# caoql98/LKGD

Hardware: AMD Instinct MI355X
Metric: denoised frames/sec (14f x 576x1024, 25-step Euler) (higher is better)
Workload: dtype f16; 1 GPU; SVD 14 frames x 576x1024, 25 Euler steps, CFG 1.0->3.0, single clip, vanilla pipeline_stable_video_diffusion_trans loop (configs[1]); unet=random-init SVD shapes (320,640,1280,1280), heads (5,10,20,20), 1.52 B params, parallelism=single GPU

## Files before the change

### include/lkgd_hip.h

```cpp
#ifndef LKGD_HIP_H
#define LKGD_HIP_H

#include <stddef.h>
#include <stdint.h>

#ifdef __cplusplus
extern "C" {
#endif

typedef void* lkgd_stream_t;

enum {
  LKGD_OK = 0,
  LKGD_E_NULL = -1,
  LKGD_E_SHAPE = -2,
  LKGD_E_ALIGN = -3,
  LKGD_E_MODE = -4,
  LKGD_E_LAUNCH = -5
};

enum { LKGD_A_PLAIN = 0, LKGD_A_CONV3X3 = 1, LKGD_A_TCONV3 = 2, LKGD_A_CONV3X3_C8 = 3, LKGD_A_CCONV3 = 4 };

typedef struct lkgd_gemm_desc {
  const void* a0;
// ... 64 lines not shown
                   float eps, const void* rowbias, int32_t ldrb, int32_t rb_d1, int32_t rb_m1, int32_t rb_d2,
                   int32_t rb_md, void* out, int32_t ldo, lkgd_stream_t stream);

int lkgd_tattn_block_c320(const void* x, int32_t ldx, const void* wstream, const float* bo, const void* rowbias, int32_t ldrb,
                          int32_t rb_d1, int32_t rb_m1, int32_t rb_d2, int32_t rb_md, int32_t rb_c0, void* out, int32_t ldo,
                          int32_t B, int32_t F, int32_t HW, float eps, lkgd_stream_t stream);

int lkgd_ln_qkv_c320(const void* x, int32_t ldx, int64_t T, const void* wstream, float eps, void* out, int32_t ldo,
                     lkgd_stream_t stream);
int lkgd_ln_qkv_c640(const void* x, int32_t ldx, int64_t T, const void* wstream, float eps, void* out, int32_t ldo,
                     lkgd_stream_t stream);

int lkgd_ff_fused_c320(const void* x, int32_t ldx, int64_t T, const void* rowbias, int32_t ldrb, int32_t rb_d1, int32_t rb_md,
                       const void* wstream, const float* b2, float eps, float s_acc, const void* res2, int32_t ldr2, float r2,
                       void* out, int32_t ldo, lkgd_stream_t stream);

int lkgd_attn_spatial(const void* q, int32_t ldq, const void* k, int32_t ldk, const void* v, int32_t ldv,
                      void* out, int32_t ldo, int32_t nbatch, int32_t S, int32_t heads, const int32_t* kv_batch_map,
                      float scale, lkgd_stream_t stream);
int lkgd_attn_spatial_qk(const void* q, int32_t ldq, const void* k, int32_t ldk, const void* v, int32_t ldv, void* out,
                         int32_t ldo, int32_t nbatch, int32_t Sq, int32_t S, int32_t heads, const int32_t* kv_batch_map,
                         float scale, lkgd_stream_t stream);

int lkgd_attn_temporal(const void* q, int32_t ldq, const void* k, int32_t ldk, const void* v, int32_t ldv,
                       void* out, int32_t ldo, int32_t B, int32_t Fq, int32_t Fk, int32_t S, int32_t heads,
                       const int32_t* kv_b_map, float scale, lkgd_stream_t stream);

int lkgd_tattn_front(const void* x, int32_t ldx, const void* wpack, const float* bqkv, void* out, int32_t ldo, int32_t B,
                     int32_t F, int32_t HW, int32_t heads, float eps, float scale, lkgd_stream_t stream);

int lkgd_prepare_unet_input(const void* latents, int32_t latents_is_f32, const void* image_latents, int32_t B,
                            int32_t F, int32_t H, int32_t W, int32_t cfg, float sigma, void* tokens_out,
                            lkgd_stream_t stream);
int lkgd_cfg_euler_step(const void* noise_tokens, void* latents, int32_t latents_is_f32, const float* guidance,
                        int32_t B, int32_t F, int32_t H, int32_t W, int32_t cfg, float sigma, float sigma_next,
                        int32_t prediction_type , lkgd_stream_t stream);
int lkgd_cfg_fusion_euler_step(const void* noise_tokens, void* latents, int32_t latents_is_f32, const float* guidance,
                               const float* weight, int32_t B, int32_t F, int32_t H, int32_t W, int32_t cfg, float sigma,
                               float sigma_next, int32_t prediction_type , lkgd_stream_t stream);
int lkgd_shard_rows(const void* src, void* dst, int32_t fl, int32_t HW, int32_t C, int32_t k, const int32_t* px, int32_t pack,
                    lkgd_stream_t stream);
int lkgd_tokens_to_nchw(const void* tokens, int32_t ld, int64_t N, int32_t C, int32_t HW, void* out,
                        lkgd_stream_t stream);
int lkgd_nchw_to_tokens(const void* nchw, int64_t N, int32_t C, int32_t HW, void* tokens, int32_t ld,
                        lkgd_stream_t stream);

// ... 65 lines not shown
```

### lkgd_amd/csrc/attn_spatial.hip

```cpp
#include "common.h"

#define KVBLK 64
#ifndef ATT_KVB16
#define ATT_KVB16 128
#endif
#ifndef ATT_NST
#define ATT_NST 2
#endif
#define ATT_THR 5.0f

__device__ __forceinline__ int k_lds_off(int row, int c) { return row * 128 + ((c ^ ((row >> 1) & 7)) << 4); }
__device__ __forceinline__ int v_lds_off(int row, int c) { return row * 128 + ((c ^ (((row >> 1) & 1) << 2)) << 4); }

template <int NW, int KVB>
__global__ __launch_bounds__(NW * 64, NW == 16 ? 1 : 2) void attn_spatial_kernel(const half_t* __restrict__ q, int ldq,
                                                              const half_t* __restrict__ k, int ldk,
                                                              const half_t* __restrict__ v, int ldv,
                                                              half_t* __restrict__ out, int ldo, int Sq, int S, int heads,
                                                              const int* __restrict__ kvmap, float scale_log2e,
                                                              int nqb, int nwg) {
  extern __shared__ __attribute__((aligned(16))) char smem[];
  const int t = threadIdx.x, lane = t & 63, w = t >> 6;
  const int h = lane >> 5, l31 = lane & 31;
  constexpr int STAGE = 2 * KVB * 128;
// ... 244 lines not shown
template <int NW, int KVB>
static int attn_launch(const void* q, int32_t ldq, const void* k, int32_t ldk, const void* v, int32_t ldv, void* out,
                       int32_t ldo, int32_t nbatch, int32_t Sq, int32_t S, int32_t heads, const int32_t* kv_batch_map, float scale,
                       hipStream_t stream) {
  constexpr int LDS = ATT_NST * 2 * KVB * 128;
  LKGD_DEVICE_ONCE_BEGIN
    if (!lkgd_dynamic_lds(LDS, attn_spatial_kernel<NW, KVB>)) return LKGD_E_LAUNCH;
  LKGD_DEVICE_ONCE_END
  const int QBLK = NW * 32;
  const int nqb = (Sq + QBLK - 1) / QBLK;
  const long long nwg = (long long)nqb * nbatch * heads;
  if (nwg > 0x7fffffffLL) return LKGD_E_SHAPE;
  hipLaunchKernelGGL((attn_spatial_kernel<NW, KVB>), dim3((unsigned)nwg), dim3(NW * 64), LDS, stream, (const half_t*)q, ldq,
                     (const half_t*)k, ldk, (const half_t*)v, ldv, (half_t*)out, ldo, Sq, S, heads, kv_batch_map,
                     scale * 1.4426950408889634f, nqb, (int)nwg);
  return hipGetLastError() == hipSuccess ? LKGD_OK : LKGD_E_LAUNCH;
}

extern "C" int lkgd_attn_spatial_qk(const void* q, int32_t ldq, const void* k, int32_t ldk, const void* v, int32_t ldv,
                                    void* out, int32_t ldo, int32_t nbatch, int32_t Sq, int32_t S, int32_t heads,
                                    const int32_t* kv_batch_map, float scale, lkgd_stream_t stream) {
  if (!q || !k || !v || !out) return LKGD_E_NULL;
  if (nbatch <= 0 || S <= 0 || Sq <= 0 || heads <= 0) return LKGD_E_SHAPE;
  if (ldq % 8 || ldk % 8 || ldv % 8 || ldo % 4) return LKGD_E_ALIGN;
  if (ldq < heads * 64 || ldk < heads * 64 || ldv < heads * 64 || ldo < heads * 64) return LKGD_E_SHAPE;
  if (!aligned16(q) || !aligned16(k) || !aligned16(v) || ((uintptr_t)out & 7)) return LKGD_E_ALIGN;
  if (attn_pipe_mode != 1 && S >= 128 && !attn_nw_override && !attn_kvb_override &&
      (attn_pipe_mode == 2 || (S >= 4096 && Sq >= 4096)))
    return lkgd_attn_pipe_launch(q, ldq, k, ldk, v, ldv, out, ldo, nbatch, Sq, S, heads, kv_batch_map, scale,
                                 (hipStream_t)stream);
  const int nw = attn_nw_override ? attn_nw_override : (Sq >= 8192 ? 16 : Sq >= 2304 ? 8 : 4);
  const int kvb = attn_kvb_override ? attn_kvb_override : (nw == 16 ? ATT_KVB16 : 64);
  hipStream_t st = (hipStream_t)stream;
#define ATT_ARGS q, ldq, k, ldk, v, ldv, out, ldo, nbatch, Sq, S, heads, kv_batch_map, scale, st
  if (nw == 16) return kvb == 128 ? attn_launch<16, 128>(ATT_ARGS) : attn_launch<16, 64>(ATT_ARGS);
  if (nw == 8) return kvb == 128 ? attn_launch<8, 128>(ATT_ARGS) : attn_launch<8, 64>(ATT_ARGS);
  return attn_launch<4, 64>(ATT_ARGS);
#undef ATT_ARGS
}

extern "C" int lkgd_attn_spatial(const void* q, int32_t ldq, const void* k, int32_t ldk, const void* v, int32_t ldv,
                                 void* out, int32_t ldo, int32_t nbatch, int32_t S, int32_t heads,
                                 const int32_t* kv_batch_map, float scale, lkgd_stream_t stream) {
  return lkgd_attn_spatial_qk(q, ldq, k, ldk, v, ldv, out, ldo, nbatch, S, S, heads, kv_batch_map, scale, stream);
}
```

### lkgd_amd/csrc/attn_spatial_pipe.hip

```cpp
#include "asm_host.h"
#include "attn_spatial_pipe.inc"
#include "attn_spatial_pipe_masked.inc"

#define AP_NW 8
#define AP_STAGE 32768
#define AP_LDS (3 * AP_STAGE)

template <int BASE>
__device__ __forceinline__ void ap_load_q(const half_t* qp, float scale_log2e) {
  for_n<4>([&](auto ks_) {
    constexpr int ks = decltype(ks_)::value;
    const half8_t raw = *(const half8_t*)(qp + ks * 16);
    half8_t sc;
#pragma unroll
    for (int e = 0; e < 8; ++e) sc[e] = (half_t)((float)raw[e] * scale_log2e);
    typedef unsigned uint4_t __attribute__((ext_vector_type(4)));
    const uint4_t u = __builtin_bit_cast(uint4_t, sc);
    agpr_write<BASE + 4 * ks + 0>(u[0]);
    agpr_write<BASE + 4 * ks + 1>(u[1]);
    agpr_write<BASE + 4 * ks + 2>(u[2]);
    agpr_write<BASE + 4 * ks + 3>(u[3]);
  });
}

template <int OBASE>
__device__ __forceinline__ void ap_store_tile(half_t* op, float inv, bool valid) {
  for_n<2>([&](auto df_) {
    constexpr int df = decltype(df_)::value;
    for_n<4>([&](auto g_) {
      constexpr int g = decltype(g_)::value;
      half4_t o;
      o[0] = (half_t)(agpr_readf<OBASE + 16 * df + 4 * g + 0>() * inv);
      o[1] = (half_t)(agpr_readf<OBASE + 16 * df + 4 * g + 1>() * inv);
      o[2] = (half_t)(agpr_readf<OBASE + 16 * df + 4 * g + 2>() * inv);
      o[3] = (half_t)(agpr_readf<OBASE + 16 * df + 4 * g + 3>() * inv);
      if (valid) *(half4_t*)(op + 32 * df + 8 * g) = o;
    });
  });
}

template <bool MASKED>
__global__ __launch_bounds__(AP_NW * 64, 1) __attribute__((amdgpu_num_vgpr(ATTN_PIPE_VEND))) void attn_pipe_kernel(
    const half_t* __restrict__ q, int ldq, const half_t* __restrict__ k, int ldk, const half_t* __restrict__ v, int ldv,
    half_t* __restrict__ out, int ldo, int Sq, int S, int heads, const int* __restrict__ kvmap, float scale_log2e, int nqb,
    int nwg) {
  extern __shared__ __attribute__((aligned(16))) char smem[];
  const int t = threadIdx.x, lane = t & 63;
  const int w = __builtin_amdgcn_readfirstlane(t >> 6);
  const int h = lane >> 5, l31 = lane & 31;

  int bid = blockIdx.x;
  {
    int xcd = bid & 7, slot = bid >> 3;
    int qq = nwg >> 3, r = nwg & 7;
    bid = (xcd < r ? xcd * (qq + 1) : r * (qq + 1) + (xcd - r) * qq) + slot;
  }
  const int bh = bid / nqb, qb = bid - bh * nqb;
  const int n = bh / heads, head = bh - n * heads;
  const int kvn = kvmap ? kvmap[n] : n;

  const half_t* kbase = k + (long long)kvn * S * ldk + head * 64;
  const half_t* vbase = v + (long long)kvn * S * ldv + head * 64;
  const int srow0 = w * 8 + (lane >> 3), sc = lane & 7;
  const int kc0 = (sc ^ ((srow0 >> 1) & 7)) * 8;
  const int vc0 = (sc ^ (((srow0 >> 1) & 1) << 2)) * 8;
  const unsigned vok = (unsigned)(srow0 * ldk + kc0) * 2u, vov = (unsigned)(srow0 * ldv + vc0) * 2u;
#pragma unroll
  for (int p = 0; p < 2; ++p) {
    char* dst = smem + (p * 64 + w * 8) * 128;
    glds16((const char*)kbase + (size_t)(p * 64) * ldk * 2 + vok, dst);
    glds16((const char*)vbase + (size_t)(p * 64) * ldv * 2 + vov, dst + 16384);
  }

  const int qrowA = qb * (AP_NW * 64) + w * 64 + l31, qrowB = qrowA + 32;
  {
    const int ra = qrowA < Sq ? qrowA : Sq - 1, rb = qrowB < Sq ? qrowB : Sq - 1;
    ap_load_q<ATTN_PIPE_QF_A>(q + ((long long)n * Sq + ra) * ldq + head * 64 + h * 8, scale_log2e);
    ap_load_q<ATTN_PIPE_QF_B>(q + ((long long)n * Sq + rb) * ldq + head * 64 + h * 8, scale_log2e);
  }

  const unsigned lds0 = (unsigned)(uintptr_t)(__attribute__((address_space(3))) char*)smem;
  unsigned ka0, ka1, ka2, ka3, va0, va1;
  {
    const int sw = (l31 >> 1) & 7;
    ka0 = lds0 + l31 * 128 + (((0 + h) ^ sw) << 4);
    ka1 = lds0 + l31 * 128 + (((2 + h) ^ sw) << 4);
    ka2 = lds0 + l31 * 128 + (((4 + h) ^ sw) << 4);
    ka3 = lds0 + l31 * 128 + (((6 + h) ^ sw) << 4);
    const int i16 = lane & 15, dgrp = (lane >> 4) & 1;
    const int tr_row = 4 * h + (i16 >> 2), tr_c = dgrp * 2 + ((i16 & 3) >> 1), tr_sub = (i16 & 1) * 8;
    const int vsw = ((tr_row >> 1) & 1) << 2;
    va0 = lds0 + tr_row * 128 + (((0 + tr_c) ^ vsw) << 4) + tr_sub;
    va1 = lds0 + tr_row * 128 + (((4 + tr_c) ^ vsw) << 4) + tr_sub;
  }
  const unsigned xora = (unsigned)((lane ^ 32) * 4);
  const unsigned hmask = h == 0 ? 0xffffu : 0u;

  const int nstages = MASKED ? (S + 127) / 128 : S / 128;
  const int dup = nstages * 128 - S;
  const int row1 = (MASKED && nstages == 2) ? S - 128 : 128;
  const unsigned long long kp = (unsigned long long)(uintptr_t)kbase + (unsigned long long)row1 * ldk * 2;
  const unsigned long long vp = (unsigned long long)(uintptr_t)vbase + (unsigned long long)row1 * ldv * 2;
  const auto [klo, khi] = sgpr_ptr(kp);
  const auto [vlo, vhi] = sgpr_ptr(vp);
  const unsigned dst1 = __builtin_amdgcn_readfirstlane(lds0 + AP_STAGE + w * 1024);
  const unsigned ldsend = __builtin_amdgcn_readfirstlane(lds0 + 3 * AP_STAGE);
  const unsigned nst = __builtin_amdgcn_readfirstlane((unsigned)nstages);
  const unsigned kp1 = __builtin_amdgcn_readfirstlane((unsigned)(64 * ldk * 2)), vp1 = __builtin_amdgcn_readfirstlane((unsigned)(64 * ldv * 2));
  const unsigned kstr = __builtin_amdgcn_readfirstlane((unsigned)(128 * ldk * 2)), vstr = __builtin_amdgcn_readfirstlane((unsigned)(128 * ldv * 2));

  float la, lb;
  if constexpr (MASKED) {
    const unsigned vm = (unsigned)l31, hm32 = h == 0 ? 0xffffffffu : 0u;
    const unsigned dupk = __builtin_amdgcn_readfirstlane((unsigned)dup);
    const unsigned klast = __builtin_amdgcn_readfirstlane((unsigned)((128 - dup) * ldk * 2));
    const unsigned vlast = __builtin_amdgcn_readfirstlane((unsigned)((128 - dup) * ldv * 2));
    asm volatile(ATTN_PIPEM_ASM
                 : [la] "=&v"(la), [lb] "=&v"(lb), [ka0] "+v"(ka0), [ka1] "+v"(ka1), [ka2] "+v"(ka2), [ka3] "+v"(ka3),
                   [va0] "+v"(va0), [va1] "+v"(va1)
                 : [vok] "v"(vok), [vov] "v"(vov), [xora] "v"(xora), [hmask] "v"(hmask), [vm] "v"(vm), [hm32] "v"(hm32), [klo] "s"(klo), [khi] "s"(khi), [vlo] "s"(vlo), [vhi] "s"(vhi),
                   [dst1] "s"(dst1), [nst] "s"(nst), [kp1] "s"(kp1), [vp1] "s"(vp1), [kstr] "s"(kstr), [vstr] "s"(vstr),
                   [ldsend] "s"(ldsend), [dup] "s"(dupk), [klast] "s"(klast), [vlast] "s"(vlast)
                 : ATTN_PIPEM_CLOBBERS);
  } else {
    asm volatile(ATTN_PIPE_ASM
                 : [la] "=&v"(la), [lb] "=&v"(lb), [ka0] "+v"(ka0), [ka1] "+v"(ka1), [ka2] "+v"(ka2), [ka3] "+v"(ka3),
                   [va0] "+v"(va0), [va1] "+v"(va1)
                 : [vok] "v"(vok), [vov] "v"(vov), [xora] "v"(xora), [hmask] "v"(hmask), [klo] "s"(klo), [khi] "s"(khi),
                   [vlo] "s"(vlo), [vhi] "s"(vhi), [dst1] "s"(dst1), [nst] "s"(nst), [kp1] "s"(kp1), [vp1] "s"(vp1),
                   [kstr] "s"(kstr), [vstr] "s"(vstr), [ldsend] "s"(ldsend)
                 : ATTN_PIPE_CLOBBERS);
  }

  int lane2;
  asm volatile("v_mbcnt_lo_u32_b32 %0, -1, 0\n\tv_mbcnt_hi_u32_b32 %0, -1, %0" : "=v"(lane2));
  const int h2 = lane2 >> 5, l2 = lane2 & 31;
  const float la_t = la + __shfl_xor(la, 32, 64), lb_t = lb + __shfl_xor(lb, 32, 64);
  const int qa = qb * (AP_NW * 64) + w * 64 + l2, qbb = qa + 32;
  const int ra2 = qa < Sq ? qa : Sq - 1, rb2 = qbb < Sq ? qbb : Sq - 1;
  ap_store_tile<ATTN_PIPE_O_A>(out + ((long long)n * Sq + ra2) * ldo + head * 64 + 4 * h2, 1.0f / la_t, qa < Sq);
  ap_store_tile<ATTN_PIPE_O_B>(out + ((long long)n * Sq + rb2) * ldo + head * 64 + 4 * h2, 1.0f / lb_t, qbb < Sq);
}

int lkgd_attn_pipe_launch(const void* q, int32_t ldq, const void* k, int32_t ldk, const void* v, int32_t ldv, void* out,
                          int32_t ldo, int32_t nbatch, int32_t Sq, int32_t S, int32_t heads, const int32_t* kv_batch_map,
                          float scale, hipStream_t stream) {
  if (S < 128) return LKGD_E_SHAPE;
  const bool masked = S % 128 != 0;
  if ((long long)64 * ldk * 2 > 0x7fffffffLL || (long long)64 * ldv * 2 > 0x7fffffffLL) return LKGD_E_SHAPE;
  LKGD_DEVICE_ONCE_BEGIN
    if (!lkgd_dynamic_lds(AP_LDS, attn_pipe_kernel<false>, attn_pipe_kernel<true>)) return LKGD_E_LAUNCH;
  LKGD_DEVICE_ONCE_END
  const int QBLK = AP_NW * 64;
  const int nqb = (Sq + QBLK - 1) / QBLK;
  const long long nwg = (long long)nqb * nbatch * heads;
  if (nwg > 0x7fffffffLL) return LKGD_E_SHAPE;
  if (masked)
    hipLaunchKernelGGL(attn_pipe_kernel<true>, dim3((unsigned)nwg), dim3(AP_NW * 64), AP_LDS, stream, (const half_t*)q, ldq,
                       (const half_t*)k, ldk, (const half_t*)v, ldv, (half_t*)out, ldo, Sq, S, heads, kv_batch_map,
                       scale * 1.4426950408889634f, nqb, (int)nwg);
  else
    hipLaunchKernelGGL(attn_pipe_kernel<false>, dim3((unsigned)nwg), dim3(AP_NW * 64), AP_LDS, stream, (const half_t*)q, ldq,
                       (const half_t*)k, ldk, (const half_t*)v, ldv, (half_t*)out, ldo, Sq, S, heads, kv_batch_map,
                       scale * 1.4426950408889634f, nqb, (int)nwg);
  return hipGetLastError() == hipSuccess ? LKGD_OK : LKGD_E_LAUNCH;
}
```

### lkgd_amd/csrc/qkv_fused.hip

```cpp
#include "asm_host.h"
#include "qkv_fused_loop.inc"
#include "qkv640_fused_loop.inc"

#define QK_WAVES 4
#define QK_LDS (QK_NSLOT * QK_SLOT)

struct qk_params {
  const half_t* x; int ldx; long long T;
  const char* wstream;
  float eps;
  half_t* out; int ldo;
  int npanels;
};

template <int C>
__global__ __launch_bounds__(QK_WAVES * 64, 1) __attribute__((amdgpu_num_vgpr(256))) void ln_qkv_kernel(qk_params p) {
  constexpr int NKS = C / 16, PARTS = NKS / 20;
  static_assert(QK_SLOT == QK6_SLOT && QK_NSLOT == QK6_NSLOT && QK_AHEAD == QK6_AHEAD && QK_ZF == 0 && QK6_ZF == 0, "one ring layout");
  extern __shared__ __attribute__((aligned(16))) char smem[];
  const int t = threadIdx.x, lane = t & 63;
  const int w = __builtin_amdgcn_readfirstlane(t >> 6);
  const int h = lane >> 5, l31 = lane & 31;
  if ((int)blockIdx.x >= p.npanels) return;

  unsigned long long ahead_bytes = 0;
#pragma unroll
  for (int c = 0; c < QK_AHEAD; ++c) {
    const char* src = p.wstream + ahead_bytes + lane * 16;
    char* dst = smem + c * QK_SLOT;
#pragma unroll
    for (int j = 0; j < 5; ++j) glds16(src + (w + 4 * j) * 1024, dst + (w + 4 * j) * 1024);
    if (c % PARTS == 0) glds16(src + 20480, dst + 20480);
    ahead_bytes += c % PARTS == 0 ? QK_W1_BYTES : QK_W2_BYTES;
  }
  const unsigned lds0 = (unsigned)(uintptr_t)(__attribute__((address_space(3))) char*)smem;
  const unsigned long long sp0 = (unsigned long long)(uintptr_t)p.wstream;
  const auto [sp0lo, sp0hi] = sgpr_ptr(sp0);
  auto [splo, sphi] = sgpr_ptr(sp0 + ahead_bytes);
  const unsigned ldsw = __builtin_amdgcn_readfirstlane(lds0 + (unsigned)w * 1024u);
  const unsigned lds0u = __builtin_amdgcn_readfirstlane(lds0);
  const unsigned fa0 = lds0 + lane * 16, fa1 = fa0 + 2 * QK_SLOT, fa2 = fa0 + 4 * QK_SLOT;
// ... 40 lines not shown
  };

  auto load_rows = [&](int panel, half8_t (&raw)[NKS]) {
    const half_t* xp = p.x + tok_of(panel) * p.ldx + 8 * h;
#pragma unroll
    for (int ks = 0; ks < NKS; ++ks) raw[ks] = *(const half8_t*)(xp + 16 * ks);
  };
  {
    half8_t raw[NKS];
    load_rows(blockIdx.x, raw);
    layernorm_rows(raw);
  }
  asm volatile("s_waitcnt vmcnt(0)" ::: "memory");
#pragma unroll 1
  for (int panel = blockIdx.x; panel < p.npanels; panel += gridDim.x) {
    const int nextp = panel + (int)gridDim.x;
    half_t* orow = p.out + tok_of(panel) * p.ldo + 8 * h;
    splo = __builtin_amdgcn_readfirstlane(splo);
    sphi = __builtin_amdgcn_readfirstlane(sphi);
    if constexpr (C == 320) {
      const half_t* xrow = p.x + tok_of(nextp < p.npanels ? nextp : panel) * p.ldx + 8 * h;
      half8_t nraw[NKS];
#define QK_ROW_OUT(i) [r##i] "=&v"(nraw[i])
      asm volatile(QK_PANEL_ASM
                   : [splo] "+s"(splo), [sphi] "+s"(sphi), QK_ROW_OUT(0), QK_ROW_OUT(1), QK_ROW_OUT(2), QK_ROW_OUT(3), QK_ROW_OUT(4),
                     QK_ROW_OUT(5), QK_ROW_OUT(6), QK_ROW_OUT(7), QK_ROW_OUT(8), QK_ROW_OUT(9), QK_ROW_OUT(10), QK_ROW_OUT(11),
                     QK_ROW_OUT(12), QK_ROW_OUT(13), QK_ROW_OUT(14), QK_ROW_OUT(15), QK_ROW_OUT(16), QK_ROW_OUT(17), QK_ROW_OUT(18),
                     QK_ROW_OUT(19)
                   : [xrow] "v"(xrow), [orow] "v"(orow), [fa0] "v"(fa0), [fa1] "v"(fa1), [fa2] "v"(fa2), [vo0] "v"(vo0), [vo1] "v"(vo1),
                     [vo2] "v"(vo2), [vo3] "v"(vo3), [vo4] "v"(vo4), [vob] "v"(vob), [hmask] "v"(hmask), [ldsw] "s"(ldsw),
                     [lds0] "s"(lds0u), [sp0lo] "s"(sp0lo), [sp0hi] "s"(sp0hi)
                   : QK_CLOBBERS);
      if (nextp < p.npanels) layernorm_rows(nraw);
    } else {
      asm volatile(QK6_PANEL_ASM
                   : [splo] "+s"(splo), [sphi] "+s"(sphi)
                   : [orow] "v"(orow), [fa0] "v"(fa0), [fa1] "v"(fa1), [fa2] "v"(fa2), [vo0] "v"(vo0), [vo1] "v"(vo1), [vo2] "v"(vo2),
                     [vo3] "v"(vo3), [vo4] "v"(vo4), [vob] "v"(vob), [hmask] "v"(hmask), [ldsw] "s"(ldsw), [lds0] "s"(lds0u),
                     [sp0lo] "s"(sp0lo), [sp0hi] "s"(sp0hi)
                   : QK6_CLOBBERS);
      half8_t nraw[NKS];
      load_rows(nextp < p.npanels ? nextp : panel, nraw);
      if (nextp < p.npanels) layernorm_rows(nraw);
    }
  }
  asm volatile("s_waitcnt vmcnt(0)" ::: "memory");
}

template <int C>
static int ln_qkv_launch(const void* x, int32_t ldx, int64_t T, const void* wstream, float eps, void* out, int32_t ldo,
                         lkgd_stream_t stream) {
  if (!x || !wstream || !out) return LKGD_E_NULL;
  if (T <= 0 || T > 0x7fffffffLL * 64) return LKGD_E_SHAPE;
  if (ldx % 8 || ldo % 8 || ldx < C || ldo < 3 * C) return LKGD_E_ALIGN;
  if (!aligned16(x) || !aligned16(wstream) || !aligned16(out)) return LKGD_E_ALIGN;
  LKGD_DEVICE_ONCE_BEGIN
    if (!lkgd_dynamic_lds(QK_LDS, ln_qkv_kernel<C>)) return LKGD_E_LAUNCH;
  LKGD_DEVICE_ONCE_END
  const int cus = lkgd_cu_count();
  const long long npanels = (T + QK_WAVES * 32 - 1) / (QK_WAVES * 32);
  qk_params p;
  p.x = (const half_t*)x; p.ldx = ldx; p.T = T; p.wstream = (const char*)wstream; p.eps = eps;
  p.out = (half_t*)out; p.ldo = ldo; p.npanels = (int)npanels;
  const int grid = npanels < cus ? (int)npanels : cus;
  hipLaunchKernelGGL(ln_qkv_kernel<C>, dim3(grid), dim3(QK_WAVES * 64), QK_LDS, (hipStream_t)stream, p);
  return hipGetLastError() == hipSuccess ? LKGD_OK : LKGD_E_LAUNCH;
}

extern "C" int lkgd_ln_qkv_c320(const void* x, int32_t ldx, int64_t T, const void* wstream, float eps, void* out, int32_t ldo,
                                lkgd_stream_t stream) {
  return ln_qkv_launch<320>(x, ldx, T, wstream, eps, out, ldo, stream);
}
extern "C" int lkgd_ln_qkv_c640(const void* x, int32_t ldx, int64_t T, const void* wstream, float eps, void* out, int32_t ldo,
                                lkgd_stream_t stream) {
  return ln_qkv_launch<640>(x, ldx, T, wstream, eps, out, ldo, stream);
}
```

### lkgd_amd/ops.py

```python
from __future__ import annotations

import ctypes as C
import os
from typing import Optional, Sequence, Tuple

import torch

from . import _lib
from ._lib import GemmDesc, check

A_PLAIN, A_CONV3X3, A_TCONV3, A_CONV3X3_C8, A_CCONV3 = 0, 1, 2, 3, 4
GEMM_TILE128, GEMM_TILE256, GEMM_STREAM, GEMM_WIDE, GEMM_ROWPANEL, GEMM_RESW, GEMM_MID = 1, 2, 3, 4, 5, 6, 7
GEMM_PROGRAMS = {"tile128": GEMM_TILE128, "tile256": GEMM_TILE256, "stream": GEMM_STREAM, "wide": GEMM_WIDE,
                 "rowpanel": GEMM_ROWPANEL, "resw": GEMM_RESW, "mid": GEMM_MID}

_zeros = {}

GEMM_EVENTS = None

import threading as _threading

_tls = _threading.local()


# ... 347 lines not shown
    _req(x, torch.float16, "x")
    if gamma is not None:
        _req(gamma, torch.float32, "gamma")
    T, C_ = x.shape
    if out is None:
        out = torch.empty(T, C_, dtype=torch.float16, device=x.device)
    d1, m1, d2, md = rowmap if rowmap is not None else (1, 0, 1, 1)
    check(_L().lkgd_layernorm(x.data_ptr(), _ld(x), T, C_, _ptr(gamma), _ptr(beta), eps,
                                    _ptr(rowbias), _ld(rowbias) if rowbias is not None else 0, d1, m1, d2, md,
                                    out.data_ptr(), _ld(out), _stream()), "lkgd_layernorm")
    return out


FF_FUSED = os.environ.get("LKGD_NO_FF_FUSED", "0") != "1"


LN_QKV = os.environ.get("LKGD_NO_LN_QKV", "0") != "1"


def ln_qkv_ok(T: int, N: int, C_: int) -> bool:
    return LN_QKV and C_ in (320, 640) and N == 3 * C_ and T >= (30000 if C_ == 640 else 60000)


def ln_qkv(x: torch.Tensor, wstream: torch.Tensor, out: torch.Tensor, eps: float = 1e-5) -> torch.Tensor:
    _req(x, torch.float16, "x"); _req(wstream, torch.float16, "wstream"); _req(out, torch.float16, "out")
    T, C_ = x.shape
    if C_ not in (320, 640):
        raise _lib.LkgdHipError("ln_qkv: 320 or 640 channels")
    _gemm_family("lkgd_ln_qkv_c320" if C_ == 320 else "lkgd_ln_qkv_c640",
                 (x.data_ptr(), _ld(x), T, wstream.data_ptr(), eps, out.data_ptr(), _ld(out)), 2.0 * T * 3 * C_ * C_)
    return out


def ff_fused_ok(C_: int, inner: int) -> bool:
    return FF_FUSED and C_ == 320 and inner == 1280


def ff_fused(x: torch.Tensor, wstream: torch.Tensor, b2: torch.Tensor, out: torch.Tensor, eps: float = 1e-5,
             rowbias: Optional[torch.Tensor] = None, rowmap: Optional[RowMap] = None, s_acc: float = 1.0,
             res2: Optional[torch.Tensor] = None, r2: float = 0.0) -> torch.Tensor:
    _req(x, torch.float16, "x"); _req(wstream, torch.float16, "wstream"); _req(b2, torch.float32, "b2")
    _req(out, torch.float16, "out")
    if x.shape[1] != 320 or out.shape != x.shape:
        raise _lib.LkgdHipError("ff_fused: x / out must be [T, 320] token matrices of the same row count")
    if res2 is not None:
        _req(res2, torch.float16, "res2")
        if res2.shape[0] != x.shape[0]:
            raise _lib.LkgdHipError("ff_fused: res2 must hold one row per token")
    if rowbias is not None:
        _req(rowbias, torch.float16, "rowbias")
    d1, m1, d2, md = (rowmap if rowmap is not None else (1, 1, 1, 1))[:4]
    if rowbias is not None and (m1 != 1 or d2 != 1 or (len(rowmap) > 4 and rowmap[4] != 0)):
        raise _lib.LkgdHipError("ff_fused: only (row // d1) % md row maps (no c0 term)")
    _gemm_family("lkgd_ff_fused_c320",
                 (x.data_ptr(), _ld(x), x.shape[0], _ptr(rowbias), _ld(rowbias) if rowbias is not None else 0, d1,
                  min(md, 1 << 30), wstream.data_ptr(), b2.data_ptr(), eps, s_acc, _ptr(res2),
                  _ld(res2) if res2 is not None else 0, r2, out.data_ptr(), _ld(out)),
                 2.0 * x.shape[0] * (2560 * 320 + 320 * 1280))
    return out


def attn_spatial(q, k, v, out, nbatch: int, S: int, heads: int, kv_batch_map: Optional[torch.Tensor] = None,
                 scale: float = 0.125, Sq: Optional[int] = None):
    _req(q, torch.float16, "q"); _req(k, torch.float16, "k"); _req(v, torch.float16, "v")
    if Sq is None or Sq == S:
        check(_L().lkgd_attn_spatial(q.data_ptr(), _ld(q), k.data_ptr(), _ld(k), v.data_ptr(), _ld(v),
                                     out.data_ptr(), _ld(out), nbatch, S, heads, _ptr(kv_batch_map), scale,
                                     _stream()), "lkgd_attn_spatial")
    else:
        check(_L().lkgd_attn_spatial_qk(q.data_ptr(), _ld(q), k.data_ptr(), _ld(k), v.data_ptr(), _ld(v),
                                        out.data_ptr(), _ld(out), nbatch, Sq, S, heads, _ptr(kv_batch_map), scale,
                                        _stream()), "lkgd_attn_spatial_qk")
    return out


def attn_temporal(q, k, v, out, B: int, F: int, S: int, heads: int, kv_b_map: Optional[torch.Tensor] = None,
                  scale: float = 0.125, Fq: Optional[int] = None):
    _req(q, torch.float16, "q"); _req(k, torch.float16, "k"); _req(v, torch.float16, "v")
    check(_L().lkgd_attn_temporal(q.data_ptr(), _ld(q), k.data_ptr(), _ld(k), v.data_ptr(), _ld(v),
                                        out.data_ptr(), _ld(out), B, Fq if Fq is not None else F, F, S, heads,
                                        _ptr(kv_b_map), scale, _stream()),
          "lkgd_attn_temporal")
    return out


def tattn_front(x: torch.Tensor, wpack: torch.Tensor, bqkv: Optional[torch.Tensor], out: torch.Tensor, B: int, F: int, HW: int,
                heads: int, eps: float = 1e-5, scale: float = 0.125) -> torch.Tensor:
    _req(x, torch.float16, "x"); _req(wpack, torch.float16, "wpack"); _req(out, torch.float16, "out")
    check(_L().lkgd_tattn_front(x.data_ptr(), _ld(x), wpack.data_ptr(), _ptr(bqkv), out.data_ptr(), _ld(out), B, F, HW, heads,
                                eps, scale, _stream()), "lkgd_tattn_front")
    return out


# ... 725 lines not shown
```

### lkgd_amd/unet.py

```python
from __future__ import annotations

import math
from dataclasses import dataclass
from types import SimpleNamespace
from typing import List, Optional, Tuple, Union

import torch
import torch.nn as nn

from . import ops
from . import replay as _replay
from . import trace as _trace
from ._lib import LkgdHipError
from .module import PackedModule
from .packing import (f32, pack_conv3x3, pack_conv3x3_c8, pack_ff_fused, pack_geglu, pack_linear, pack_ln_proj, pack_tblock,
                      pack_tconv3, pack_tfront)

TIME_CONTEXT_ORDER = "interleaved_0_27"

RESNET_EPS = {
    "CrossAttnDownBlockSpatioTemporal": 1e-6,
    "DownBlockSpatioTemporal": 1e-5,
    "UNetMidBlockSpatioTemporal": 1e-5,
    "UpBlockSpatioTemporal": 1e-6,
# ... 189 lines not shown
    _gemm_runs(ctx, a, out, lambda i: (*_part(vs[i], part, Cc), table(i)), rowmap=cross[1] if cross is not None else None,
               res1=res1, rows=rows, **epilogue)


def _part(v, part: str, Cc: int):
    if part == "out":
        return v.wo, v.bo
    if part == "joint":
        return v.jw, v.jb
    if part == "qkv":
        return v.wqkv, v.bqkv
    return (v.wqkv[:Cc], v.bqkv[:Cc]) if part == "q" else (v.wqkv[Cc:], v.bqkv[Cc:])


def _first_use(pk, name: str, build):
    v = getattr(pk, name, None)
    if v is None:
        with _replay.invariant():
            v = build()
        setattr(pk, name, v)
    return v


def _ln_qkv(block, x: torch.Tensor, qkv: torch.Tensor) -> None:
    a1 = block._pk.a1
    ops.ln_qkv(x, _first_use(a1, "wlnqkv", lambda: pack_ln_proj(a1.wqkv, a1.bqkv)), qkv)


def _self_qkv(block, ctx: "Ctx", h: torch.Tensor, keep_ln: bool):
    T, Cc = h.shape
    fused = ctx.lora is None and not keep_ln and ops.ln_qkv_ok(T, 3 * Cc, Cc)
    ln = None if fused else ops.layernorm(h, None, None, 1e-5)
    qkv = ctx.new(T, 3 * Cc)
    if fused:
        _ln_qkv(block, h, qkv)
    else:
        _project(block, ctx, "a1", "qkv", ln, qkv)
    return qkv, ln


def _attend_temporal(block, ctx: "Ctx", which: str, a: torch.Tensor, geom, *, rows: Optional[int] = None, kv_b_map=None,
                     ln_fused: bool = False) -> torch.Tensor:
    T, Cc = a.shape
    qkv = ctx.new(T, 3 * Cc)
    if ln_fused:
        _ln_qkv(block, a, qkv)
    else:
        _project(block, ctx, which, "qkv", a, qkv, rows=rows)
    att = ctx.new(T, Cc)
    heads = (block.attn1 if which == "a1" else block.attn1n).heads
    ops.attn_temporal(qkv[:, :Cc], qkv[:, Cc:2 * Cc], qkv[:, 2 * Cc:], att, *geom, heads, kv_b_map=kv_b_map)
    return att


def temporal_path(C_: int, heads: int, F: int, F_total: int, HW: int, T: int, frame_shards: int, *, lora: bool, joint: bool,
                  gather: bool):
    if F_total != F:
        return ("pixels", False) if (not gather and HW >= frame_shards) else ("gather", True)
    if not lora and ops.tattn_front_ok(C_, heads, F, HW):
        if ops.tattn_block_ok(C_, heads, F, HW):
            return "block", joint
# ... 124 lines not shown
        self.attn1 = Attention(dim, None, num_attention_heads, attention_head_dim)
        self.norm2 = nn.LayerNorm(dim, eps=1e-5)
        self.attn2 = Attention(dim, cross_attention_dim, num_attention_heads, attention_head_dim)
        self.norm3 = nn.LayerNorm(dim, eps=1e-5)
        self.ff = FeedForward(dim)
        self.enable_joint_attention = False
        self.joint_scale = 1.0

    def pack(self, model):
        pk = SimpleNamespace(a1=self.attn1.pack_self(self.norm1), ff=self.ff.pack(self.norm3))
        pk.xoff = model._register_cross(self.attn2)
        if hasattr(self, "attn1n"):
            pk.a1n = self.attn1n.pack_self(self.norm1)
            _pack_joint_post(self, pk, spatial=True)
        if hasattr(self, "conv_fuse"):
            pk.wfuse, pk.bfuse = pack_conv3x3(self.conv_fuse.weight), f32(self.conv_fuse.bias)
        pk.var = {}
        self._pk = pk

    @_trace.traced("spatial_transformer_block")
    def run(self, ctx: Ctx, h: torch.Tensor) -> torch.Tensor:
        T, Cc = h.shape
        joint = self.enable_joint_attention and hasattr(self, "attn1n")
        qkv, ln = _self_qkv(self, ctx, h, keep_ln=joint)
        pre = self._joint_start(ctx, ln) if (joint and ctx.flip_mirror) else None
        att = ctx.new(T, Cc)
        ops.attn_spatial(qkv[:, :Cc], qkv[:, Cc:2 * Cc], qkv[:, 2 * Cc:], att, ctx.N, ctx.HW, self.attn1.heads)
        h1 = ctx.new(T, Cc)
        if getattr(self, "_lkgd_fsm", False) and self.enable_joint_attention:
            if ctx.lora is not None:
                raise LkgdHipError("masked LoRA together with the FSM hook is not supported")
            _project(self, ctx, "a1", "out", att, h1, res1=h)
            return self._tail(ctx, self._fsm(ctx, h1))
        _project(self, ctx, "a1", "out", att, h1, cross=(ctx.b0, ops.rowmap_div(ctx.F * ctx.HW)), res1=h)
        if joint:
            h1 = self._joint(ctx, ln, h1, pre)
        return self._tail(ctx, h1)

    def _tail(self, ctx: Ctx, h1: torch.Tensor) -> torch.Tensor:
        if ctx.cross_Lk > 1:
            h1 = _cross_literal(self, ctx, h1, ops.rowmap_div(ctx.F * ctx.HW), ctx.b0)
        return _ff_ln(ctx, self._pk.ff, h1)

    def _joint_start(self, ctx: Ctx, ln: torch.Tensor):
        T, Cc = ln.shape
        if ctx.spatial_partner is None:
            raise LkgdHipError("joint attention enabled but no joint_attn_mask set (patch.set_joint_attention_mask)")
        qkv = ctx.new(T, 3 * Cc)
        _project(self, ctx, "a1n", "qkv", ln, qkv)
        kk, vv, finish = qkv[:, Cc:2 * Cc], qkv[:, 2 * Cc:], None
# ... 976 lines not shown
```

Measured before the change: 6.136 frames/s.

## Emit V in MFMA fragment order from fused LN-QKV for spatial attention

The fused layernorm+QKV kernel for C=320 can now write V into a separate contiguous plane laid out in the attention kernel's fragment order, with Q and K packed at ldo=640. A new VFRAG variant of the pipelined spatial attention kernel reads that plane directly, so V loads are contiguous and the LDS transpose/swizzle addressing for V is simplified. This targets V load and LDS transposition overhead in the highest-resolution spatial self-attention. It adds new assembly inner loops, applies only to unmasked S%128==0 shapes with C=320, and can be disabled with an environment variable.

```diff
diff --git a/include/lkgd_hip.h b/include/lkgd_hip.h
--- a/include/lkgd_hip.h
+++ b/include/lkgd_hip.h
@@ -110,6 +110,19 @@
                          int32_t ldo, int32_t nbatch, int32_t Sq, int32_t S, int32_t heads, const int32_t* kv_batch_map,
                          float scale, lkgd_stream_t stream);
 
+enum { LKGD_LDV_FRAGMENTS = -1 };
+#if defined(__HIP__)
+#define LKGD_HOST_DEVICE __attribute__((host)) __attribute__((device))
+#else
+#define LKGD_HOST_DEVICE
+#endif
+static inline LKGD_HOST_DEVICE int64_t lkgd_vfrag_index(int64_t token, int32_t channel, int32_t heads) {
+  const int64_t g = token >> 4;
+  const int32_t r = (int32_t)(token & 15), head = channel >> 6, half = (channel >> 5) & 1, c = channel & 31;
+  const int32_t hh = (r >> 2) & 1, e = (r & 3) + 4 * (r >> 3);
+  return ((((g * heads + head) * 2 + half) * 64 + 32 * hh + c) << 3) + e;
+}
+
 int lkgd_attn_temporal(const void* q, int32_t ldq, const void* k, int32_t ldk, const void* v, int32_t ldv,
                        void* out, int32_t ldo, int32_t B, int32_t Fq, int32_t Fk, int32_t S, int32_t heads,
                        const int32_t* kv_b_map, float scale, lkgd_stream_t stream);
diff --git a/lkgd_amd/csrc/attn_spatial.hip b/lkgd_amd/csrc/attn_spatial.hip
--- a/lkgd_amd/csrc/attn_spatial.hip
+++ b/lkgd_amd/csrc/attn_spatial.hip
@@ -290,9 +290,13 @@
                                     const int32_t* kv_batch_map, float scale, lkgd_stream_t stream) {
   if (!q || !k || !v || !out) return LKGD_E_NULL;
   if (nbatch <= 0 || S <= 0 || Sq <= 0 || heads <= 0) return LKGD_E_SHAPE;
-  if (ldq % 8 || ldk % 8 || ldv % 8 || ldo % 4) return LKGD_E_ALIGN;
-  if (ldq < heads * 64 || ldk < heads * 64 || ldv < heads * 64 || ldo < heads * 64) return LKGD_E_SHAPE;
+  const bool vfrag = ldv == LKGD_LDV_FRAGMENTS;
+  if (ldq % 8 || ldk % 8 || (!vfrag && ldv % 8) || ldo % 4) return LKGD_E_ALIGN;
+  if (ldq < heads * 64 || ldk < heads * 64 || (!vfrag && ldv < heads * 64) || ldo < heads * 64) return LKGD_E_SHAPE;
   if (!aligned16(q) || !aligned16(k) || !aligned16(v) || ((uintptr_t)out & 7)) return LKGD_E_ALIGN;
+  if (vfrag)
+    return S % 128 ? LKGD_E_SHAPE
+                   : lkgd_attn_pipe_launch(q, ldq, k, ldk, v, ldv, out, ldo, nbatch, Sq, S, heads, kv_batch_map, scale, (hipStream_t)stream);
   if (attn_pipe_mode != 1 && S >= 128 && !attn_nw_override && !attn_kvb_override &&
       (attn_pipe_mode == 2 || (S >= 4096 && Sq >= 4096)))
     return lkgd_attn_pipe_launch(q, ldq, k, ldk, v, ldv, out, ldo, nbatch, Sq, S, heads, kv_batch_map, scale,
diff --git a/lkgd_amd/csrc/attn_spatial_pipe.hip b/lkgd_amd/csrc/attn_spatial_pipe.hip
--- a/lkgd_amd/csrc/attn_spatial_pipe.hip
+++ b/lkgd_amd/csrc/attn_spatial_pipe.hip
@@ -1,6 +1,7 @@
 #include "asm_host.h"
 #include "attn_spatial_pipe.inc"
 #include "attn_spatial_pipe_masked.inc"
+#include "vfrag/attn_spatial_pipe_vfrag.inc"
 
 #define AP_NW 8
 #define AP_STAGE 32768
@@ -39,7 +40,7 @@
   });
 }
 
-template <bool MASKED>
+template <bool MASKED, bool VFRAG>
 __global__ __launch_bounds__(AP_NW * 64, 1) __attribute__((amdgpu_num_vgpr(ATTN_PIPE_VEND))) void attn_pipe_kernel(
     const half_t* __restrict__ q, int ldq, const half_t* __restrict__ k, int ldk, const half_t* __restrict__ v, int ldv,
     half_t* __restrict__ out, int ldo, int Sq, int S, int heads, const int* __restrict__ kvmap, float scale_log2e, int nqb,
@@ -60,16 +61,21 @@
   const int kvn = kvmap ? kvmap[n] : n;
 
   const half_t* kbase = k + (long long)kvn * S * ldk + head * 64;
-  const half_t* vbase = v + (long long)kvn * S * ldv + head * 64;
+  static_assert(!(MASKED && VFRAG), "the fragment-order plane comes in whole stages");
+  const half_t* vbase = VFRAG ? v + lkgd_vfrag_index((long long)kvn * S, head * 64, heads) : v + (long long)kvn * S * ldv + head * 64;
   const int srow0 = w * 8 + (lane >> 3), sc = lane & 7;
   const int kc0 = (sc ^ ((srow0 >> 1) & 7)) * 8;
   const int vc0 = (sc ^ (((srow0 >> 1) & 1) << 2)) * 8;
-  const unsigned vok = (unsigned)(srow0 * ldk + kc0) * 2u, vov = (unsigned)(srow0 * ldv + vc0) * 2u;
+  const unsigned vok = (unsigned)(srow0 * ldk + kc0) * 2u;
+  const unsigned vov = VFRAG ? (unsigned)lkgd_vfrag_index(16 * (w >> 1) + 4 * h, 32 * (w & 1) + l31, heads) * 2u
+                             : (unsigned)(srow0 * ldv + vc0) * 2u;
+  const unsigned vhalf = VFRAG ? (unsigned)lkgd_vfrag_index(64, 0, heads) * 2u : (unsigned)(64 * ldv * 2);
+  const unsigned vstage = VFRAG ? (unsigned)lkgd_vfrag_index(128, 0, heads) * 2u : (unsigned)(128 * ldv * 2);
 #pragma unroll
   for (int p = 0; p < 2; ++p) {
     char* dst = smem + (p * 64 + w * 8) * 128;
     glds16((const char*)kbase + (size_t)(p * 64) * ldk * 2 + vok, dst);
-    glds16((const char*)vbase + (size_t)(p * 64) * ldv * 2 + vov, dst + 16384);
+    glds16((const char*)vbase + (size_t)p * vhalf + vov, dst + 16384);
   }
 
   const int qrowA = qb * (AP_NW * 64) + w * 64 + l31, qrowB = qrowA + 32;
@@ -90,7 +96,7 @@
     const int i16 = lane & 15, dgrp = (lane >> 4) & 1;
     const int tr_row = 4 * h + (i16 >> 2), tr_c = dgrp * 2 + ((i16 & 3) >> 1), tr_sub = (i16 & 1) * 8;
     const int vsw = ((tr_row >> 1) & 1) << 2;
-    va0 = lds0 + tr_row * 128 + (((0 + tr_c) ^ vsw) << 4) + tr_sub;
+    va0 = VFRAG ? lds0 + lane * 16 : lds0 + tr_row * 128 + (((0 + tr_c) ^ vsw) << 4) + tr_sub;
     va1 = lds0 + tr_row * 128 + (((4 + tr_c) ^ vsw) << 4) + tr_sub;
   }
   const unsigned xora = (unsigned)((lane ^ 32) * 4);
@@ -100,14 +106,14 @@
   const int dup = nstages * 128 - S;
   const int row1 = (MASKED && nstages == 2) ? S - 128 : 128;
   const unsigned long long kp = (unsigned long long)(uintptr_t)kbase + (unsigned long long)row1 * ldk * 2;
-  const unsigned long long vp = (unsigned long long)(uintptr_t)vbase + (unsigned long long)row1 * ldv * 2;
+  const unsigned long long vp = (unsigned long long)(uintptr_t)vbase + (VFRAG ? (unsigned long long)vstage : (unsigned long long)row1 * ldv * 2);
   const auto [klo, khi] = sgpr_ptr(kp);
   const auto [vlo, vhi] = sgpr_ptr(vp);
   const unsigned dst1 = __builtin_amdgcn_readfirstlane(lds0 + AP_STAGE + w * 1024);
   const unsigned ldsend = __builtin_amdgcn_readfirstlane(lds0 + 3 * AP_STAGE);
   const unsigned nst = __builtin_amdgcn_readfirstlane((unsigned)nstages);
-  const unsigned kp1 = __builtin_amdgcn_readfirstlane((unsigned)(64 * ldk * 2)), vp1 = __builtin_amdgcn_readfirstlane((unsigned)(64 * ldv * 2));
-  const unsigned kstr = __builtin_amdgcn_readfirstlane((unsigned)(128 * ldk * 2)), vstr = __builtin_amdgcn_readfirstlane((unsigned)(128 * ldv * 2));
+  const unsigned kp1 = __builtin_amdgcn_readfirstlane((unsigned)(64 * ldk * 2)), vp1 = __builtin_amdgcn_readfirstlane(vhalf);
+  const unsigned kstr = __builtin_amdgcn_readfirstlane((unsigned)(128 * ldk * 2)), vstr = __builtin_amdgcn_readfirstlane(vstage);
 
   float la, lb;
   if constexpr (MASKED) {
@@ -122,6 +128,13 @@
                    [dst1] "s"(dst1), [nst] "s"(nst), [kp1] "s"(kp1), [vp1] "s"(vp1), [kstr] "s"(kstr), [vstr] "s"(vstr),
                    [ldsend] "s"(ldsend), [dup] "s"(dupk), [klast] "s"(klast), [vlast] "s"(vlast)
                  : ATTN_PIPEM_CLOBBERS);
+  } else if constexpr (VFRAG) {
+    asm volatile(ATTN_PIPEF_ASM
+                 : [la] "=&v"(la), [lb] "=&v"(lb), [ka0] "+v"(ka0), [ka1] "+v"(ka1), [ka2] "+v"(ka2), [ka3] "+v"(ka3), [va0] "+v"(va0)
+                 : [vok] "v"(vok), [vov] "v"(vov), [xora] "v"(xora), [hmask] "v"(hmask), [klo] "s"(klo), [khi] "s"(khi),
+                   [vlo] "s"(vlo), [vhi] "s"(vhi), [dst1] "s"(dst1), [nst] "s"(nst), [kp1] "s"(kp1), [vp1] "s"(vp1),
+                   [kstr] "s"(kstr), [vstr] "s"(vstr), [ldsend] "s"(ldsend)
+                 : ATTN_PIPEF_CLOBBERS);
   } else {
     asm volatile(ATTN_PIPE_ASM
                  : [la] "=&v"(la), [lb] "=&v"(lb), [ka0] "+v"(ka0), [ka1] "+v"(ka1), [ka2] "+v"(ka2), [ka3] "+v"(ka3),
@@ -147,20 +160,27 @@
                           float scale, hipStream_t stream) {
   if (S < 128) return LKGD_E_SHAPE;
   const bool masked = S % 128 != 0;
-  if ((long long)64 * ldk * 2 > 0x7fffffffLL || (long long)64 * ldv * 2 > 0x7fffffffLL) return LKGD_E_SHAPE;
+  const bool vfrag = ldv == LKGD_LDV_FRAGMENTS;
+  if (vfrag && masked) return LKGD_E_SHAPE;
+  if ((long long)64 * ldk * 2 > 0x7fffffffLL || (long long)64 * (vfrag ? 64 * heads : ldv) * 2 > 0x7fffffffLL) return LKGD_E_SHAPE;
   LKGD_DEVICE_ONCE_BEGIN
-    if (!lkgd_dynamic_lds(AP_LDS, attn_pipe_kernel<false>, attn_pipe_kernel<true>)) return LKGD_E_LAUNCH;
+    if (!lkgd_dynamic_lds(AP_LDS, attn_pipe_kernel<false, false>, attn_pipe_kernel<true, false>, attn_pipe_kernel<false, true>))
+      return LKGD_E_LAUNCH;
   LKGD_DEVICE_ONCE_END
   const int QBLK = AP_NW * 64;
   const int nqb = (Sq + QBLK - 1) / QBLK;
   const long long nwg = (long long)nqb * nbatch * heads;
   if (nwg > 0x7fffffffLL) return LKGD_E_SHAPE;
-  if (masked)
-    hipLaunchKernelGGL(attn_pipe_kernel<true>, dim3((unsigned)nwg), dim3(AP_NW * 64), AP_LDS, stream, (const half_t*)q, ldq,
+  if (vfrag)
+    hipLaunchKernelGGL((attn_pipe_kernel<false, true>), dim3((unsigned)nwg), dim3(AP_NW * 64), AP_LDS, stream, (const half_t*)q, ldq,
+                       (const half_t*)k, ldk, (const half_t*)v, ldv, (half_t*)out, ldo, Sq, S, heads, kv_batch_map,
+                       scale * 1.4426950408889634f, nqb, (int)nwg);
+  else if (masked)
+    hipLaunchKernelGGL((attn_pipe_kernel<true, false>), dim3((unsigned)nwg), dim3(AP_NW * 64), AP_LDS, stream, (const half_t*)q, ldq,
                        (const half_t*)k, ldk, (const half_t*)v, ldv, (half_t*)out, ldo, Sq, S, heads, kv_batch_map,
                        scale * 1.4426950408889634f, nqb, (int)nwg);
   else
-    hipLaunchKernelGGL(attn_pipe_kernel<false>, dim3((unsigned)nwg), dim3(AP_NW * 64), AP_LDS, stream, (const half_t*)q, ldq,
+    hipLaunchKernelGGL((attn_pipe_kernel<false, false>), dim3((unsigned)nwg), dim3(AP_NW * 64), AP_LDS, stream, (const half_t*)q, ldq,
                        (const half_t*)k, ldk, (const half_t*)v, ldv, (half_t*)out, ldo, Sq, S, heads, kv_batch_map,
                        scale * 1.4426950408889634f, nqb, (int)nwg);
   return hipGetLastError() == hipSuccess ? LKGD_OK : LKGD_E_LAUNCH;
diff --git a/lkgd_amd/csrc/qkv_fused.hip b/lkgd_amd/csrc/qkv_fused.hip
--- a/lkgd_amd/csrc/qkv_fused.hip
+++ b/lkgd_amd/csrc/qkv_fused.hip
@@ -1,6 +1,7 @@
 #include "asm_host.h"
 #include "qkv_fused_loop.inc"
 #include "qkv640_fused_loop.inc"
+#include "vfrag/qkv_fused_loop_vfrag.inc"
 
 #define QK_WAVES 4
 #define QK_LDS (QK_NSLOT * QK_SLOT)
@@ -11,12 +12,16 @@
   float eps;
   half_t* out; int ldo;
   int npanels;
+  half_t* vplane;
 };
 
-template <int C>
+template <int C, bool VFRAG>
 __global__ __launch_bounds__(QK_WAVES * 64, 1) __attribute__((amdgpu_num_vgpr(256))) void ln_qkv_kernel(qk_params p) {
   constexpr int NKS = C / 16, PARTS = NKS / 20;
+  static_assert(!VFRAG || C == 320, "the fragment-order statement exists for C = 320");
   static_assert(QK_SLOT == QK6_SLOT && QK_NSLOT == QK6_NSLOT && QK_AHEAD == QK6_AHEAD && QK_ZF == 0 && QK6_ZF == 0, "one ring layout");
+  static_assert(QK_SLOT == QKF_SLOT && QK_NSLOT == QKF_NSLOT && QK_AHEAD == QKF_AHEAD && QKF_ZF == 0 && QK_W1_BYTES == QKF_W1_BYTES &&
+                QK_W2_BYTES == QKF_W2_BYTES, "one ring layout, one stream");
   extern __shared__ __attribute__((aligned(16))) char smem[];
   const int t = threadIdx.x, lane = t & 63;
   const int w = __builtin_amdgcn_readfirstlane(t >> 6);
@@ -103,15 +108,28 @@
       const half_t* xrow = p.x + tok_of(nextp < p.npanels ? nextp : panel) * p.ldx + 8 * h;
       half8_t nraw[NKS];
 #define QK_ROW_OUT(i) [r##i] "=&v"(nraw[i])
-      asm volatile(QK_PANEL_ASM
-                   : [splo] "+s"(splo), [sphi] "+s"(sphi), QK_ROW_OUT(0), QK_ROW_OUT(1), QK_ROW_OUT(2), QK_ROW_OUT(3), QK_ROW_OUT(4),
-                     QK_ROW_OUT(5), QK_ROW_OUT(6), QK_ROW_OUT(7), QK_ROW_OUT(8), QK_ROW_OUT(9), QK_ROW_OUT(10), QK_ROW_OUT(11),
-                     QK_ROW_OUT(12), QK_ROW_OUT(13), QK_ROW_OUT(14), QK_ROW_OUT(15), QK_ROW_OUT(16), QK_ROW_OUT(17), QK_ROW_OUT(18),
-                     QK_ROW_OUT(19)
-                   : [xrow] "v"(xrow), [orow] "v"(orow), [fa0] "v"(fa0), [fa1] "v"(fa1), [fa2] "v"(fa2), [vo0] "v"(vo0), [vo1] "v"(vo1),
-                     [vo2] "v"(vo2), [vo3] "v"(vo3), [vo4] "v"(vo4), [vob] "v"(vob), [hmask] "v"(hmask), [ldsw] "s"(ldsw),
-                     [lds0] "s"(lds0u), [sp0lo] "s"(sp0lo), [sp0hi] "s"(sp0hi)
-                   : QK_CLOBBERS);
+#define QK_ROWS_OUT                                                                                                              \
+  QK_ROW_OUT(0), QK_ROW_OUT(1), QK_ROW_OUT(2), QK_ROW_OUT(3), QK_ROW_OUT(4), QK_ROW_OUT(5), QK_ROW_OUT(6), QK_ROW_OUT(7),        \
+  QK_ROW_OUT(8), QK_ROW_OUT(9), QK_ROW_OUT(10), QK_ROW_OUT(11), QK_ROW_OUT(12), QK_ROW_OUT(13), QK_ROW_OUT(14), QK_ROW_OUT(15),  \
+  QK_ROW_OUT(16), QK_ROW_OUT(17), QK_ROW_OUT(18), QK_ROW_OUT(19)
+      if constexpr (VFRAG) {
+        const long long tb = (long long)panel * (QK_WAVES * 32) + w * 32;
+        const char* vb0 = (const char*)(p.vplane + lkgd_vfrag_index(tb + 4 * h, l31, C / 64)) + 4096;
+        const char *vb1 = vb0 + 8192, *vb2 = vb0 + 16384;
+        asm volatile(QKF_PANEL_ASM
+                     : [splo] "+s"(splo), [sphi] "+s"(sphi), QK_ROWS_OUT
+                     : [xrow] "v"(xrow), [orow] "v"(orow), [fa0] "v"(fa0), [fa1] "v"(fa1), [fa2] "v"(fa2), [vo0] "v"(vo0), [vo1] "v"(vo1),
+                       [vo2] "v"(vo2), [vo3] "v"(vo3), [vo4] "v"(vo4), [vob] "v"(vob), [hmask] "v"(hmask), [vb0] "v"(vb0), [vb1] "v"(vb1),
+                       [vb2] "v"(vb2), [ldsw] "s"(ldsw), [lds0] "s"(lds0u), [sp0lo] "s"(sp0lo), [sp0hi] "s"(sp0hi)
+                     : QKF_CLOBBERS);
+      } else {
+        asm volatile(QK_PANEL_ASM
+                     : [splo] "+s"(splo), [sphi] "+s"(sphi), QK_ROWS_OUT
+                     : [xrow] "v"(xrow), [orow] "v"(orow), [fa0] "v"(fa0), [fa1] "v"(fa1), [fa2] "v"(fa2), [vo0] "v"(vo0), [vo1] "v"(vo1),
+                       [vo2] "v"(vo2), [vo3] "v"(vo3), [vo4] "v"(vo4), [vob] "v"(vob), [hmask] "v"(hmask), [ldsw] "s"(ldsw),
+                       [lds0] "s"(lds0u), [sp0lo] "s"(sp0lo), [sp0hi] "s"(sp0hi)
+                     : QK_CLOBBERS);
+      }
       if (nextp < p.npanels) layernorm_rows(nraw);
     } else {
       asm volatile(QK6_PANEL_ASM
@@ -133,18 +151,27 @@
                          lkgd_stream_t stream) {
   if (!x || !wstream || !out) return LKGD_E_NULL;
   if (T <= 0 || T > 0x7fffffffLL * 64) return LKGD_E_SHAPE;
-  if (ldx % 8 || ldo % 8 || ldx < C || ldo < 3 * C) return LKGD_E_ALIGN;
+  const bool vfrag = ldo < 0;
+  if (vfrag) {
+    if (C != 320 || ldo == INT32_MIN || T % (QK_WAVES * 32)) return LKGD_E_SHAPE;
+    ldo = -ldo;
+  }
+  if (ldx % 8 || ldo % 8 || ldx < C || ldo < (vfrag ? 2 : 3) * C) return LKGD_E_ALIGN;
   if (!aligned16(x) || !aligned16(wstream) || !aligned16(out)) return LKGD_E_ALIGN;
   LKGD_DEVICE_ONCE_BEGIN
-    if (!lkgd_dynamic_lds(QK_LDS, ln_qkv_kernel<C>)) return LKGD_E_LAUNCH;
+    if (!lkgd_dynamic_lds(QK_LDS, ln_qkv_kernel<C, false>, ln_qkv_kernel<320, true>)) return LKGD_E_LAUNCH;
   LKGD_DEVICE_ONCE_END
   const int cus = lkgd_cu_count();
   const long long npanels = (T + QK_WAVES * 32 - 1) / (QK_WAVES * 32);
   qk_params p;
   p.x = (const half_t*)x; p.ldx = ldx; p.T = T; p.wstream = (const char*)wstream; p.eps = eps;
   p.out = (half_t*)out; p.ldo = ldo; p.npanels = (int)npanels;
+  p.vplane = vfrag ? (half_t*)out + T * ldo : nullptr;
   const int grid = npanels < cus ? (int)npanels : cus;
-  hipLaunchKernelGGL(ln_qkv_kernel<C>, dim3(grid), dim3(QK_WAVES * 64), QK_LDS, (hipStream_t)stream, p);
+  if (vfrag)
+    hipLaunchKernelGGL((ln_qkv_kernel<320, true>), dim3(grid), dim3(QK_WAVES * 64), QK_LDS, (hipStream_t)stream, p);
+  else
+    hipLaunchKernelGGL((ln_qkv_kernel<C, false>), dim3(grid), dim3(QK_WAVES * 64), QK_LDS, (hipStream_t)stream, p);
   return hipGetLastError() == hipSuccess ? LKGD_OK : LKGD_E_LAUNCH;
 }
 
diff --git a/lkgd_amd/ops.py b/lkgd_amd/ops.py
--- a/lkgd_amd/ops.py
+++ b/lkgd_amd/ops.py
@@ -393,13 +393,40 @@
     return LN_QKV and C_ in (320, 640) and N == 3 * C_ and T >= (30000 if C_ == 640 else 60000)
 
 
-def ln_qkv(x: torch.Tensor, wstream: torch.Tensor, out: torch.Tensor, eps: float = 1e-5) -> torch.Tensor:
+LDV_FRAGMENTS = -1
+
+ATTN_VFRAG = os.environ.get("LKGD_NO_ATTN_VFRAG", "0") != "1"
+
+
+def attn_vfrag_ok(C_: int, heads: int, S: int) -> bool:
+    return ATTN_VFRAG and C_ == 320 and heads * 64 == C_ and S % 128 == 0 and S >= 4096
+
+
+def vfrag_index(token, channel, heads: int):
+    g, r = token >> 4, token & 15
+    head, half, c = channel >> 6, (channel >> 5) & 1, channel & 31
+    hh, e = (r >> 2) & 1, (r & 3) + 4 * (r >> 3)
+    return ((((g * heads + head) * 2 + half) * 64 + 32 * hh + c) << 3) + e
+
+
+def vfrag_split(out: torch.Tensor):
+    T, C3 = out.shape
+    flat = out.view(-1)
+    return flat[:T * (C3 // 3) * 2].view(T, 2 * (C3 // 3)), flat[T * (C3 // 3) * 2:]
+
+
+def ln_qkv(x: torch.Tensor, wstream: torch.Tensor, out: torch.Tensor, eps: float = 1e-5, v_fragments: bool = False) -> torch.Tensor:
     _req(x, torch.float16, "x"); _req(wstream, torch.float16, "wstream"); _req(out, torch.float16, "out")
     T, C_ = x.shape
     if C_ not in (320, 640):
         raise _lib.LkgdHipError("ln_qkv: 320 or 640 channels")
+    ldo = _ld(out)
+    if v_fragments:
+        if C_ != 320 or T % 128 or tuple(out.shape) != (T, 3 * C_) or not out.is_contiguous():
+            raise _lib.LkgdHipError("ln_qkv: the fragment-V form needs C = 320, T % 128 == 0 and a contiguous [T, 960] out")
+        ldo = -2 * C_
     _gemm_family("lkgd_ln_qkv_c320" if C_ == 320 else "lkgd_ln_qkv_c640",
-                 (x.data_ptr(), _ld(x), T, wstream.data_ptr(), eps, out.data_ptr(), _ld(out)), 2.0 * T * 3 * C_ * C_)
+                 (x.data_ptr(), _ld(x), T, wstream.data_ptr(), eps, out.data_ptr(), ldo), 2.0 * T * 3 * C_ * C_)
     return out
 
 
@@ -432,14 +459,20 @@
 
 
 def attn_spatial(q, k, v, out, nbatch: int, S: int, heads: int, kv_batch_map: Optional[torch.Tensor] = None,
-                 scale: float = 0.125, Sq: Optional[int] = None):
+                 scale: float = 0.125, Sq: Optional[int] = None, v_fragments: bool = False):
     _req(q, torch.float16, "q"); _req(k, torch.float16, "k"); _req(v, torch.float16, "v")
+    if v_fragments:
+        if v.dim() != 1 or not v.is_contiguous() or v.numel() % (S * heads * 64) or S % 128:
+            raise _lib.LkgdHipError("attn_spatial: the fragment-order V is one contiguous plane of whole batch entries, S % 128 == 0")
+        _ld_v = lambda t: LDV_FRAGMENTS
+    else:
+        _ld_v = _ld
     if Sq is None or Sq == S:
-        check(_L().lkgd_attn_spatial(q.data_ptr(), _ld(q), k.data_ptr(), _ld(k), v.data_ptr(), _ld(v),
+        check(_L().lkgd_attn_spatial(q.data_ptr(), _ld(q), k.data_ptr(), _ld(k), v.data_ptr(), _ld_v(v),
                                      out.data_ptr(), _ld(out), nbatch, S, heads, _ptr(kv_batch_map), scale,
                                      _stream()), "lkgd_attn_spatial")
     else:
-        check(_L().lkgd_attn_spatial_qk(q.data_ptr(), _ld(q), k.data_ptr(), _ld(k), v.data_ptr(), _ld(v),
+        check(_L().lkgd_attn_spatial_qk(q.data_ptr(), _ld(q), k.data_ptr(), _ld(k), v.data_ptr(), _ld_v(v),
                                         out.data_ptr(), _ld(out), nbatch, Sq, S, heads, _ptr(kv_batch_map), scale,
                                         _stream()), "lkgd_attn_spatial_qk")
     return out
diff --git a/lkgd_amd/unet.py b/lkgd_amd/unet.py
--- a/lkgd_amd/unet.py
+++ b/lkgd_amd/unet.py
@@ -235,21 +235,21 @@
     return v
 
 
-def _ln_qkv(block, x: torch.Tensor, qkv: torch.Tensor) -> None:
+def _ln_qkv(block, x: torch.Tensor, qkv: torch.Tensor, v_fragments: bool = False) -> None:
     a1 = block._pk.a1
-    ops.ln_qkv(x, _first_use(a1, "wlnqkv", lambda: pack_ln_proj(a1.wqkv, a1.bqkv)), qkv)
-
-
-def _self_qkv(block, ctx: "Ctx", h: torch.Tensor, keep_ln: bool):
+    ops.ln_qkv(x, _first_use(a1, "wlnqkv", lambda: pack_ln_proj(a1.wqkv, a1.bqkv)), qkv, v_fragments=v_fragments)
+
+
+def _self_qkv(block, ctx: "Ctx", h: torch.Tensor, keep_ln: bool, v_fragments: bool = False):
     T, Cc = h.shape
     fused = ctx.lora is None and not keep_ln and ops.ln_qkv_ok(T, 3 * Cc, Cc)
     ln = None if fused else ops.layernorm(h, None, None, 1e-5)
     qkv = ctx.new(T, 3 * Cc)
     if fused:
-        _ln_qkv(block, h, qkv)
+        _ln_qkv(block, h, qkv, v_fragments=v_fragments)
     else:
         _project(block, ctx, "a1", "qkv", ln, qkv)
-    return qkv, ln
+    return qkv, ln, fused and v_fragments
 
 
 def _attend_temporal(block, ctx: "Ctx", which: str, a: torch.Tensor, geom, *, rows: Optional[int] = None, kv_b_map=None,
@@ -420,10 +420,16 @@
     def run(self, ctx: Ctx, h: torch.Tensor) -> torch.Tensor:
         T, Cc = h.shape
         joint = self.enable_joint_attention and hasattr(self, "attn1n")
-        qkv, ln = _self_qkv(self, ctx, h, keep_ln=joint)
+        vfrag = (not joint and not getattr(self, "_lkgd_fsm", False) and ctx.shard is None
+                 and ops.attn_vfrag_ok(Cc, self.attn1.heads, ctx.HW))
+        qkv, ln, vfrag = _self_qkv(self, ctx, h, keep_ln=joint, v_fragments=vfrag)
         pre = self._joint_start(ctx, ln) if (joint and ctx.flip_mirror) else None
         att = ctx.new(T, Cc)
-        ops.attn_spatial(qkv[:, :Cc], qkv[:, Cc:2 * Cc], qkv[:, 2 * Cc:], att, ctx.N, ctx.HW, self.attn1.heads)
+        if vfrag:
+            qk, vplane = ops.vfrag_split(qkv)
+            ops.attn_spatial(qk[:, :Cc], qk[:, Cc:], vplane, att, ctx.N, ctx.HW, self.attn1.heads, v_fragments=True)
+        else:
+            ops.attn_spatial(qkv[:, :Cc], qkv[:, Cc:2 * Cc], qkv[:, 2 * Cc:], att, ctx.N, ctx.HW, self.attn1.heads)
         h1 = ctx.new(T, Cc)
         if getattr(self, "_lkgd_fsm", False) and self.enable_joint_attention:
             if ctx.lora is not None:
```

After: 6.148 frames/s, median of 6. Within noise of the previous version (+0.2%).
